# imazen/image-webp

Measured on AMD Instinct MI355X. Metric: 1920x1080 lossy encodes/s (Q75, method 4), higher is better.
Workload: dtype int32; 1 GPU; encode_frame_lossy 1920x1080 RGBA Q75 m4; device_batch=1024, distinct_frames=4, mbs_per_frame=8160, parallelism=frames sharded over 1 GPU(s), steps_pipelined=True, pipeline_lanes=2

## Files before the change

### image-webp_amd/csrc/zw_enc_kernels.hip

```cpp
#include "zw_dev.h"

#include <type_traits>

#include "zw_enc_rows.h"

#ifdef ZW_NW
#define ZW_NW1 ZW_NW
#define ZW_NW2 ZW_NW
#endif
#ifndef ZW_NW1
#define ZW_NW1 12
#endif
#ifndef ZW_NW2
#define ZW_NW2 12
#endif
#define NW_MAX (ZW_NW1 > ZW_NW2 ? ZW_NW1 : ZW_NW2)
#ifndef ZW_DYN_PRIO
#define ZW_DYN_PRIO 1
#endif
#ifndef ZW_DYN_PRIO1
#define ZW_DYN_PRIO1 2
#endif
#ifndef ZW_P1_LUMA_MAX
#define ZW_P1_LUMA_MAX 3
// ... 467 lines not shown
            for (int i = 0; i < 4; i++) accum[i] = dacc[i] = 0;
            int cc = 0;
            for (int a = min_a; a <= max_a; a++) {
                if (H[a] > 0) {
                    while (cc + 1 < 4) {
                        int dc = iabs(a - centers[cc]), dn = iabs(a - centers[cc + 1]);
                        if (dn < dc) cc++;
                        else break;
                    }
                    map[a] = (uint8_t)cc;
                    dacc[cc] += (uint32_t)a * H[a];
                    accum[cc] += H[a];
                }
            }
            int displaced = 0;
            wa = 0;
            tw = 0;
            for (int n = 0; n < 4; n++) {
                if (accum[n] > 0) {
                    uint8_t nc = (uint8_t)((dacc[n] + accum[n] / 2) / accum[n]);
                    displaced += iabs(centers[n] - nc);
                    centers[n] = nc;
                    wa += (int)nc * (int)accum[n];
                    tw += accum[n];
                }
            }
            if (displaced < 5) break;
        }
        int mid = tw > 0 ? (wa + (int)tw / 2) / (int)tw : 128;
        int minc = centers[0], maxc = centers[0];
        for (int i = 1; i < 4; i++) {
            minc = min(minc, (int)centers[i]);
            maxc = max(maxc, (int)centers[i]);
        }
        int rng = maxc == minc ? 1 : maxc - minc;
        for (int s = 0; s < 4; s++) {
            int ta = 255 * ((int)centers[s] - mid) / rng;
            ta = ta < -127 ? -127 : (ta > 127 ? 127 : ta);
            int sq = segment_quant(base, ta, 50);
            int delta = (int)(int8_t)((int8_t)sq - (int8_t)base);
            segment_init(P.seg[s], sq, delta);
        }
        uint32_t cnt[4] = {0, 0, 0, 0};
        for (int a = 0; a < 256; a++) cnt[map[a]] += H[a];
        uint32_t t01 = cnt[0] + cnt[1], t23 = cnt[2] + cnt[3];
#define GETP(a, b) ((a) + (b) == 0 ? 255 : (uint8_t)((255 * (a) + ((a) + (b)) / 2) / ((a) + (b))))
        P.seg_probs[0] = GETP(t01, t23);
        P.seg_probs[1] = GETP(cnt[0], cnt[1]);
        P.seg_probs[2] = GETP(cnt[2], cnt[3]);
#undef GETP
        P.seg_update_map = P.seg_probs[0] != 255 || P.seg_probs[1] != 255 || P.seg_probs[2] != 255;
        P.seg_enabled = 1;
    }
    params[f] = P;
    uint4* Hz = (uint4*)(histo + (size_t)f * 256);
    for (int i = 0; i < 64; i++) Hz[i] = make_uint4(0u, 0u, 0u, 0u);
}

struct EncArgs {
    const uint8_t *Y, *U, *V;
    const uint8_t* alpha;
    const ZwFrameParams* params;
    const ZwLevelCosts* lcost;
    int8_t* derr;
    ZwMbOut* out;
    uint8_t *ry, *ru, *rv;
    size_t ysz, csz;
    int mbw, mbh, pass;
    int* dbg;
    uint8_t* rows;
    uint32_t* sizes;
    int nframes;
};

struct MbLds {
    uint8_t sy[256], su[64], sv[64];
    uint8_t ws[17 * ZW_BPS];
    uint8_t left_y[20], left_u[12], left_v[12], left_c[12];
    int8_t left_derr[4];
    uint8_t modes[16];
    int16_t lev[25][16];
};

struct WaveLds {
    MbLds mb;
    uint8_t cu[9 * ZW_BPS], cv[9 * ZW_BPS];
    uint32_t uvc[64][8];
    int dc[64];
    int y2d[64];
    int y2cost[4];
    int V[2][40];
    int nzt[4], nzl[4];
    int misc[16];
    uint32_t pst[2][4];
    uint8_t win_y[32], win_u[8], win_v[8], win_c[12];
    int8_t win_d[4];
#ifdef ZW_PHASE_PROF
    unsigned long long ph[24];
#endif
};


struct Ctx {
    const EncArgs* a;
    const ZwFrameParams* P;
    int method;
    const ZwSegment* S;
    const ZwSegment* Sl;
    const LdsTables* T;
    WaveLds* W;
    MbLds* M;
    uint8_t *top_y, *top_u, *top_v, *top_c;
    int8_t* top_derr;
    const uint8_t *srcY, *srcU, *srcV;
    const uint8_t *sY, *sU, *sV;
    int ys, cs;
    int mbx, mby, lane, seg;
    int f;
    int oy, oc, ocx, od;
};

__device__ void build_luma_border(const Ctx& C, int part = 2)
{
    uint8_t* ws = C.M->ws;
    const int l = C.lane;
    const int mbw = C.a->mbw;
    const bool want = part == 2 || (part == 0 ? (l < 17 || l >= 32) : (l >= 17 && l < 32));
    if (!want) {
    } else if (l < 32) {
        int v;
        if (l == 0) v = C.mby == 0 ? 127 : (C.mbx == 0 ? 129 : C.M->left_y[0]);
        else if (C.mby == 0) v = 127;
        else if (l <= 16) v = C.top_y[C.oy + l - 1];
        else if (C.mbx == mbw - 1) v = C.top_y[C.oy + 15];
        else v = C.top_y[C.oy + l - 1];
        ws[l] = (uint8_t)v;
        if (l >= 17 && l < 21) {
            ws[4 * ZW_BPS + l] = (uint8_t)v;
            ws[8 * ZW_BPS + l] = (uint8_t)v;
            ws[12 * ZW_BPS + l] = (uint8_t)v;
        }
    } else if (l < 48) {
        int i = l - 32;
        ws[(i + 1) * ZW_BPS] = C.mbx == 0 ? 129 : C.M->left_y[1 + i];
    }
    wsync();
}

__device__ void build_chroma_border(const Ctx& C)
{
    const int l = C.lane;
    if (l < 34) {
        const int pl = l >= 17;
        const int i = pl ? l - 17 : l;
        uint8_t* w = pl ? C.W->cv : C.W->cu;
        const uint8_t* top = pl ? C.top_v : C.top_u;
        const uint8_t* left = pl ? C.M->left_v : C.M->left_u;
        if (i == 0) w[0] = C.mby == 0 ? 127 : (C.mbx == 0 ? 129 : left[0]);
        else if (i <= 8) w[i] = C.mby == 0 ? 127 : top[C.oc + i - 1];
        else w[(i - 8) * ZW_BPS] = C.mbx == 0 ? 129 : left[i - 8];
    }
    wsync();
}

template <int PASS>
__device__ void pick_i16(const Ctx& C, int& best_mode, unsigned long long& best_score)
{
    const int lane = C.lane, m = lane >> 4, b = lane & 15, bx = b & 3, by = b >> 2;
    const uint8_t* ws = C.M->ws;
    const ZwSegment& S = *C.S;
    const LdsTables* T = C.T;
    const int above = C.mby != 0, left = C.mbx != 0;
    int dcv;
    {
        const int top = lane < 16;
        const int v = (int)ws[csel(top, 1 + b, (b + 1) * ZW_BPS)] & -(int)(lane < 32 && (top ? above : left));
        const int sum = red16(v);
        const int s = __builtin_amdgcn_readlane(sum, 0) + __builtin_amdgcn_readlane(sum, 16);
        const int shf = 3 + above + left;
        dcv = (!above && !left) ? 128 : ((s + (1 << (shf - 1))) >> shf);
    }
    int src[16], pr[16], r[16], c[16];
    {
        const int P0 = ws[0];
        int L[4], Tp[4];
#pragma unroll
        for (int i = 0; i < 4; i++) {
            L[i] = ws[(by * 4 + i + 1) * ZW_BPS];
            Tp[i] = ws[1 + bx * 4 + i];
        }
#pragma unroll
        for (int i = 0; i < 4; i++) {
            const uint32_t srow = *(const uint32_t*)(C.sY + (by * 4 + i) * 16 + bx * 4);
#pragma unroll
            for (int j = 0; j < 4; j++) {
                const int p = sel4(m, dcv, Tp[j], L[i], clamp255(L[i] + Tp[j] - P0));
                const int sv = (int)((srow >> (8 * j)) & 255u);
                src[i * 4 + j] = sv;
                pr[i * 4 + j] = p;
                r[i * 4 + j] = sv - p;
            }
        }
    }
    fdct16_pk(r, c);
    int aq[16], dq[16];
    aq[0] = 0;
    int nzac = 0;
#pragma unroll
    for (int k = 1; k < 16; k++) {
        aq[k] = (int)((__umul24((uint32_t)iabs(c[k]), S.y1.iq[1]) + S.y1.bias[1]) >> 17);
        nzac |= aq[k];
        dq[k] = m24(c[k] < 0 ? -aq[k] : aq[k], (int)S.y1.q[1]);
    }
    nzac = nzac != 0;
    int cost = (int)rcost_bf<1, PASS == 2>(aq, 0, 0, T);
    int y2cost;
    {
        const int d = wht_g(c[0], b);
        const int t = b > 0;
        const int ay = (int)((__umul24((uint32_t)iabs(d), S.y2.iq[t]) + S.y2.bias[t]) >> 17);
        const int qy = d < 0 ? -ay : ay;
        y2cost = (int)rcost_g<0, PASS == 2>(qy, b, 0, 1, T);
        dq[0] = iwht_g(m24(qy, (int)S.y2.q[t]), b);
    }
    idct16(dq);
    int rec[16], sse = 0, flat = 1;
    const int s00 = C.sY[0];
#pragma unroll
    for (int k = 0; k < 16; k++) {
        rec[k] = clamp255(pr[k] + dq[k]);
        const int d = src[k] - rec[k];
        sse += m24(d, d);
        flat &= src[k] == s00;
    }
    int td = iabs(ttransform_diff_pk(rec, src)) >> 5;
    sse = red16(sse);
    td = red16(td);
    cost = red16(cost);
    nzac = red16(nzac);
    flat = red16(flat);
    const int srcflat = __builtin_amdgcn_readlane(flat, 0) == 16;
    cost += y2cost;
    int sd = S.tlambda > 0 ? ((int)S.tlambda * td + 128) >> 8 : 0;
    int dfin = sse;
    if (srcflat && nzac == 0) {
        dfin = sse * 2;
        sd = sd * 2;
    }
    const int mcost = sel4(m, d_FIXED_COSTS_I16[0], d_FIXED_COSTS_I16[1], d_FIXED_COSTS_I16[2], d_FIXED_COSTS_I16[3]) + cost;
    const int dist = dfin + sd;
    long long brd = 0x7fffffffffffffffLL, bfin = 0;
    int bm = 0;
#pragma unroll
    for (int mm = 0; mm < 4; mm++) {
        const long long mc = __builtin_amdgcn_readlane(mcost, mm * 16);
        const long long dd = 256LL * __builtin_amdgcn_readlane(dist, mm * 16);
        const long long r_m = mc * (long long)S.l_i16 + dd;
        const long long f_m = mc * (long long)S.l_mode + dd;
        const int avail = mm == 0 || (mm == 1 && above) || (mm == 2 && left) || (mm == 3 && above && left);
        if (avail && r_m < brd) {
            brd = r_m;
            bfin = f_m;
            bm = mm;
        }
    }
    best_mode = bm;
    best_score = bfin < 0 ? 0ull : (unsigned long long)bfin;
}

#ifdef ZW_PHASE_PROF
__device__ unsigned long long zw_phase_cycles_dev[2][24];
__device__ unsigned long long zw_wave_cycles_dev[2][16][24];
#define PH_START() long long ph_t_ = clock64()
#define PH_RESET() (ph_t_ = clock64())
#define PH_MARK(k) PH_MARK_L(k, lane, PASS)
#define PH_MARK_L(k, ln, ps)                                                        \
    do {                                                                            \
        const long long n_ = clock64();                                             \
        if ((ln) == 0) C.W->ph[k] += (unsigned long long)(n_ - ph_t_);               \
        ph_t_ = n_;                                                                 \
    } while (0)
extern "C" int zw_wave_cycles(unsigned long long* out, int reset)
{
    if (hipMemcpyFromSymbol(out, HIP_SYMBOL(zw_wave_cycles_dev), sizeof(zw_wave_cycles_dev)) != hipSuccess) return -1;
    if (reset) {
        static unsigned long long z[2][16][24];
        if (hipMemcpyToSymbol(HIP_SYMBOL(zw_wave_cycles_dev), z, sizeof z) != hipSuccess) return -1;
    }
    return 0;
}
extern "C" int zw_phase_cycles(unsigned long long* out, int reset)
{
    if (hipMemcpyFromSymbol(out, HIP_SYMBOL(zw_phase_cycles_dev), sizeof(zw_phase_cycles_dev)) != hipSuccess) return -1;
    if (reset) {
        static unsigned long long z[2][24];
        if (hipMemcpyToSymbol(HIP_SYMBOL(zw_phase_cycles_dev), z, sizeof z) != hipSuccess) return -1;
    }
    return 0;
}
#define PH_COUNT(k) \
    do {                \
        if (C.lane == 0) C.W->ph[k] += 1; \
    } while (0)
#elif defined(ZW_ASM_MARKS)
#define PH_COUNT(k) (void)0
#define PH_START() asm volatile("; ZWMARK start" ::: "memory")
#define PH_RESET() (void)0
#define PH_MARK(k) asm volatile("; ZWMARK " #k ::: "memory")
#define PH_MARK_L(k, ln, ps) asm volatile("; ZWMARK " #k ::: "memory")
#else
#define PH_COUNT(k) (void)0
#define PH_START() (void)0
#define PH_RESET() (void)0
#define PH_MARK(k) (void)0
#define PH_MARK_L(k, ln, ps) (void)0
#endif

template <int NB>
__device__ __forceinline__ void i4_values_n(const Ctx& C, const int* x0, const int* y0)
{
    WaveLds* W = C.W;
    const uint8_t* ws = C.M->ws;
    const int l = C.lane;
    const int t = (int)(l >= 13) + (int)(l >= 24) + (int)(l >= 36) + (int)(l >= 37);
    const int k = min(l - 13 * (int)(l >= 13) - 11 * (int)(l >= 24), 12);
    const int t3 = (int)(t == 3), t4 = (int)(t >= 4), t12 = (int)(t == 1 || t == 2);
    const int ka = k + t3 * (11 - k) + t4 * (1 - k);
    const int kb = k + t12 + t3 * (12 - k) - t4 * k;
    const int kc = min(k + 2 * (int)(t == 1), 12);
    const int wb = 2 * (int)(t == 1) + (int)(t == 2) + 3 * (t3 + t4);
    const int wc = (int)(t == 1);
    const int sh = (int)(t != 0) + (int)(t != 0 && t != 2);
    const int oa = csel(ka < 4, -ka * ZW_BPS, ka - 4 - 4 * ZW_BPS);
    const int ob = csel(kb < 4, -kb * ZW_BPS, kb - 4 - 4 * ZW_BPS);
    const int oc = csel(kc < 4, -kc * ZW_BPS, kc - 4 - 4 * ZW_BPS);
    const bool dcl = l < 4 || (l >= 5 && l < 9);
    int v[NB], ea[NB];
#pragma unroll
    for (int h = 0; h < NB; h++) {
        const int rowL = (y0[h] + 3) * ZW_BPS + x0[h] - 1;
        ea[h] = ws[rowL + oa];
        const int eb = ws[rowL + ob], ec = ws[rowL + oc];
        v[h] = (ea[h] + wb * eb + wc * ec + ((1 << sh) >> 1)) >> sh;
    }
#pragma unroll
    for (int h = 0; h < NB; h++) {
        const int dsum = red16(dcl ? ea[h] : 0);
        if (l < 38) W->V[h][l] = v[h];
        if (l == 0) W->V[h][38] = (dsum + 4) >> 3;
    }
// ... 906 lines not shown
    const unsigned long long win = __ballot(key2 == kmin);
    const uint32_t pk = (rate & 0xffffu) | ((uint32_t)mcost << 16) | ((uint32_t)(last >= 0) << 31);
    PH_MARK_L(12, l, 0);
#pragma unroll
    for (int mb = 0; mb < 2; mb++) {
        const ZwSegment& S = *(mb ? CB : CA).S;
        MbLds* M = (mb ? CB : CA).M;
#pragma unroll
        for (int h = 0; h < NB; h++) {
            const int gg = 2 * mb + h;
            const int bk = __builtin_ctz((uint32_t)(win >> (16 * gg)) & 0xffffu) >> 2;
            const int bmode = (int)((modes >> (16 * gg + 4 * bk)) & 15ull);
            const int wl = 16 * gg + 4 * bk;
            const uint32_t bsse = (uint32_t)__builtin_amdgcn_readlane(sse, wl);
            const uint32_t bpk = (uint32_t)__builtin_amdgcn_readlane((int)pk, wl);
            const uint32_t brate = bpk & 0xffffu;
            const int bnz = (int)(bpk >> 31);
            const int i = sby[h] * 4 + sbx[h];
            I4State& s = st[mb];
            s.tnz = (s.tnz & ~(1u << sbx[h])) | ((uint32_t)bnz << sbx[h]);
            s.lnz = (s.lnz & ~(1u << sby[h])) | ((uint32_t)bnz << sby[h]);
            s.nzm |= (uint32_t)bnz << i;
            s.total_mc += (bpk >> 16) & 0x7fffu;
            s.running += rdscore(bsse, brate, S.l_mode);
            s.mpack |= (unsigned long long)bmode << (4 * i);
            if (act[mb] && l == gg) M->modes[i] = (uint8_t)bmode;
        }
    }
    const int bks = __builtin_ctz((uint32_t)(win >> (16 * g)) & 0xffffu) >> 2;
    if (k == bks && ((l >> 4) & 1) < NB && (hm ? act[1] : act[0])) {
        MbLds* M = hm ? CB.M : CA.M;
        const int xo = csel(slot, x0[sl], x0[0]), yo = csel(slot, y0[sl], y0[0]);
        const uint32_t wd = __builtin_amdgcn_perm(r32, r01, 0x04060200u);
        uint8_t* p = M->ws + (yo + q) * ZW_BPS + xo;
#pragma unroll
        for (int j = 0; j < 4; j++) p[j] = (uint8_t)(wd >> (8 * j));
        if (keep) {
            int16_t* lvp = M->lev[by * 4 + bx];
#pragma unroll
            for (int r = 0; r < 4; r++) lvp[izz_of(4 * r + q)] = (int16_t)lv[r];
        }
    }
    wsync();
    PH_MARK_L(13, l, 0);
}

template <int PASS>
__device__ uint32_t pick_i4_pair(const Ctx& CA, const Ctx& CB, unsigned long long i16A, unsigned long long i16B,
                                 bool actA, bool actB, bool keep, uint32_t& nzA, uint32_t& nzB)
{
    const int K = CA.method <= 3 ? 3 : 4;
    I4State st[2];
    st[0].running = 211ull * CA.S->l_mode;
    st[1].running = 211ull * CB.S->l_mode;
#pragma unroll
    for (int mb = 0; mb < 2; mb++) {
        st[mb].total_mc = 0;
        st[mb].mpack = 0;
        st[mb].tnz = st[mb].lnz = st[mb].nzm = 0;
    }
    bool act[2] = {actA, actB};
    const unsigned long long lim[2] = {i16A, i16B};
    I4PLane LC;
    i4p_lane_init(CA, CB, LC);
    for (int s = 0; s < 10; s++) {
        const int sbyA = s < 4 ? 0 : (s - 2) >> 1;
        const int sbxA = s - 2 * sbyA;
        if (s >= 2 && s <= 7) {
            const int bx[2] = {sbxA, sbxA - 2}, by[2] = {sbyA, sbyA + 1};
            i4p_step<PASS, 2>(CA, CB, bx, by, K, LC, st, act, keep);
        } else {
            i4p_step<PASS, 1>(CA, CB, &sbxA, &sbyA, K, LC, st, act, keep);
        }
#pragma unroll
        for (int mb = 0; mb < 2; mb++)
            if (st[mb].running >= lim[mb] || st[mb].total_mc > 256u * 16u * 16u / 4u) act[mb] = false;
        if (!act[0] && !act[1]) return 0;
    }
    nzA = st[0].nzm;
    nzB = st[1].nzm;
    return (uint32_t)act[0] | ((uint32_t)act[1] << 1);
}

__device__ int final_luma(const Ctx& C, int mode, bool trel, int y_nz_out[16], int i4_nzm)
{
    WaveLds* W = C.W;
    const ZwSegment& S = *C.S;
    const int l = C.lane;
    int anynz = 0;
    PH_START();
    if (mode == 4 && i4_nzm >= 0) {
#pragma unroll
        for (int i = 0; i < 16; i++) y_nz_out[i] = (i4_nzm >> i) & 1;
        if (l < 16) C.M->lev[16][l] = 0;
        wsync();
        PH_MARK_L(15, l, 0);
        PH_COUNT(7);
        return i4_nzm != 0;
    }
    if (mode != 4) {
        build_luma_border(C);
        const uint8_t* ws = C.M->ws;
        const int above = C.mby != 0, left = C.mbx != 0;
        const int b = l & 15, bx = b & 3, by = b >> 2;
        int dcv;
        {
            const int top = l < 16;
            const int v = (int)ws[csel(top, 1 + b, (b + 1) * ZW_BPS)] & -(int)(l < 32 && (top ? above : left));
            const int sum = red16(v);
            const int su = __builtin_amdgcn_readlane(sum, 0) + __builtin_amdgcn_readlane(sum, 16);
            const int shf = 3 + above + left;
            dcv = (!above && !left) ? 128 : ((su + (1 << (shf - 1))) >> shf);
        }
        int c[16], pr[16];
        {
            const int P0 = ws[0];
            int L[4], Tp[4], r[16];
#pragma unroll
            for (int i = 0; i < 4; i++) {
                L[i] = ws[(by * 4 + i + 1) * ZW_BPS];
                Tp[i] = ws[1 + bx * 4 + i];
            }
#pragma unroll
            for (int i = 0; i < 4; i++) {
                const uint32_t srow = *(const uint32_t*)(C.sY + (by * 4 + i) * 16 + bx * 4);
#pragma unroll
                for (int j = 0; j < 4; j++) {
                    const int p = sel4(mode, dcv, Tp[j], L[i], clamp255(L[i] + Tp[j] - P0));
                    pr[i * 4 + j] = p;
                    r[i * 4 + j] = (int)((srow >> (8 * j)) & 255u) - p;
                }
            }
            fdct16_pk(r, c);
        }
        int y2dq;
        {
            const int d = wht_g(c[0], b);
            const int t = b > 0;
            const int y2q = quantz(d, S.y2.iq[t], S.y2.bias[t]);
            if (l < 16) C.M->lev[16][izz_of(b)] = (int16_t)y2q;
            if (gmask(y2q != 0)) anynz = 1;
            y2dq = iwht_g(m24(y2q, (int)S.y2.q[t]), b);
        }
        PH_MARK_L(16, l, 0);
        int dq[16], lv[16];
        int nzb = 0;
        {
            int snz = 0;
            if (l < 16) {
#pragma unroll
                for (int k = 1; k < 16; k++) snz |= quantz(c[k], S.y1.iq[1], S.y1.bias[1]) != 0;
            }
            anynz |= __any(snz) ? 1 : 0;
        }
        if (trel) {
            int tnz = 0;
            if (l < 48) {
#pragma unroll
                for (int k = 0; k < 16; k++) dq[k] = c[k];
                tnz = trellis<1, true>(dq, lv, S.y1, S.sharpen, S.lt_i16, C.T, 0, l >> 4);
            }
            PH_MARK_L(17, l, 0);
            const unsigned long long nzm = __ballot(l < 48 && tnz);
            int nt[4], nl[4];
#pragma unroll
            for (int q = 0; q < 4; q++) {
                nt[q] = __builtin_amdgcn_readfirstlane(C.top_c[C.ocx + 1 + q]);
                nl[q] = __builtin_amdgcn_readfirstlane(C.M->left_c[1 + q]);
            }
            unsigned code = 0, nzbits = 0;
#pragma unroll
            for (int bb = 0; bb < 16; bb++) {
                const int cx = min(nl[bb >> 2] + nt[bb & 3], 2);
                const int z = (int)((nzm >> (cx * 16 + bb)) & 1ull);
                nt[bb & 3] = z;
                nl[bb >> 2] = z;
                code |= (unsigned)cx << (2 * bb);
                nzbits |= (unsigned)z << bb;
            }
            const int srcl = (int)((code >> (2 * b)) & 3u) * 16 + b;
            lv[0] = 0;
#pragma unroll
            for (int i = 0; i < 8; i++) {
                const uint32_t w = (uint32_t)__shfl((int)pack_lo(lv[2 * i], lv[2 * i + 1]), srcl);
                lv[2 * i] = lo16(w);
                lv[2 * i + 1] = hi16(w);
            }
#pragma unroll
            for (int n = 1; n < 16; n++) dq[kZZ(n)] = m24(lv[n], (int)S.y1.q[1]);
            nzb = (nzbits >> b) & 1u;
            PH_MARK_L(18, l, 0);
        } else if (l < 16) {
#pragma unroll
            for (int n = 1; n < 16; n++) {
                const int j = kZZ(n);
                lv[n] = quantz(c[j], S.y1.iq[1], S.y1.bias[1]);
                nzb |= lv[n] != 0;
            }
            dq[0] = 0;
#pragma unroll
            for (int n = 1; n < 16; n++) dq[kZZ(n)] = m24(lv[n], (int)S.y1.q[1]);
        }
        wsync();
        if (l < 16) {
            lv[0] = 0;
#pragma unroll
            for (int n = 0; n < 16; n++) C.M->lev[b][n] = (int16_t)lv[n];
            dq[0] = y2dq;
            idct16(dq);
            uint8_t* wsp = C.M->ws;
#pragma unroll
            for (int k = 0; k < 16; k++) {
                const int y = by * 4 + (k >> 2), x = bx * 4 + (k & 3);
                wsp[(y + 1) * ZW_BPS + 1 + x] = (uint8_t)clamp255(pr[k] + dq[k]);
            }
        }
        const unsigned nzmask = (unsigned)__ballot(l < 16 && nzb);
        for (int k = 0; k < 16; k++) y_nz_out[k] = (int)((nzmask >> k) & 1u);
        wsync();
        PH_MARK_L(14, l, 0);
    } else {
        build_luma_border(C);
        int top_nz[4], left_nz[4];
        for (int k = 0; k < 4; k++) {
            top_nz[k] = C.top_c[C.ocx + 1 + k];
            left_nz[k] = C.M->left_c[1 + k];
        }
        for (int i = 0; i < 16; i++) {
            const int sby = i >> 2, sbx = i & 3, x0 = sbx * 4 + 1, y0 = sby * 4 + 1;
            const int bm = C.M->modes[i];
            i4_values(C, x0, y0);
            const int k = l & 15;
            const int pk = i4_pred_at(W->V[0], i4_src_index(C.T, bm, k), W->V[0][5 + (k & 3)] - W->V[0][4]);
            const int svk = C.sY[(sby * 4 + (k >> 2)) * 16 + sbx * 4 + (k & 3)];
            const int ck = fdct_g(svk - pk, k);
            const int ctx0 = min(left_nz[sby] + top_nz[sbx], 2);
            if (C.a->dbg && C.a->pass == 2 && l < 16) {
                int* d = C.a->dbg + (((size_t)C.f * C.a->mbw * C.a->mbh + (size_t)C.mby * C.a->mbw + C.mbx) * 16 + i) * 34;
                d[k] = ck;
                d[16 + k] = pk;
                if (k == 0) {
                    d[32] = ctx0;
                    d[33] = bm;
                }
            }
            const int qs = quantz(ck, S.y1.iq[k > 0], S.y1.bias[k > 0]);
            const int snz = gmask(qs != 0) != 0;
            int dqk, nzq;
            if (trel) {
                const int cn = gget(ck, zz_of(k));
                int lvn;
                nzq = trellis_g<0>(cn, k, S.y1, S.sharpen, S.lt_i4, C.T, 3, ctx0, lvn);
                if (l < 16) C.M->lev[i][k] = (int16_t)lvn;
                dqk = m24(gget(lvn, izz_of(k)), (int)S.y1.q[k > 0]);
            } else {
                if (l < 16) C.M->lev[i][izz_of(k)] = (int16_t)qs;
                nzq = snz;
                dqk = m24(qs, (int)S.y1.q[k > 0]);
            }
            const int rk = idct_g(dqk, k);
            if (l < 16) C.M->ws[(y0 + (k >> 2)) * ZW_BPS + x0 + (k & 3)] = (uint8_t)clamp255(pk + rk);
            wsync();
            if (l == 0) {
                W->misc[1] = nzq;
                W->misc[2] = snz;
            }
            wsync();
            const int nz = W->misc[1];
            anynz |= W->misc[2];
            top_nz[sbx] = nz;
            left_nz[sby] = nz;
            y_nz_out[i] = nz;
            wsync();
        }
        if (l < 16) C.M->lev[16][l] = 0;
        wsync();
        PH_MARK_L(15, l, 0);
        PH_COUNT(7);
    }
    return anynz;
}

__device__ int final_chroma(const Ctx& C, int mode, int8_t* top_derr, int uv_nz[8])
{
    WaveLds* W = C.W;
    const ZwSegment& S = *C.S;
    const int l = C.lane;
    const int h = l >> 5, b = l & 7, pl = b >> 2, bx = b & 1, by = (b >> 1) & 1;
    const bool act = (l & 31) < 8;
    int cf[2][4];
    uint32_t p01[2], p32[2];
    {
        const uint32_t* e = W->uvc[h * 32 + mode * 8 + b];
#pragma unroll
        for (int c = 0; c < 2; c++) {
            cf[c][0] = lo16(e[2 * c]);
            cf[c][1] = hi16(e[2 * c]);
            cf[c][2] = lo16(e[2 * c + 1]);
            cf[c][3] = hi16(e[2 * c + 1]);
        }
        p01[0] = e[4];
        p32[0] = e[5];
        p01[1] = e[6];
        p32[1] = e[7];
    }
    {
        const int q = (int)S.uv.q[0];
        const uint32_t iq = S.uv.iq[0], bias = S.uv.bias[0];
        const uint32_t zt = S.uv.zthresh[0];
        int dcs[8];
#pragma unroll
        for (int k = 0; k < 8; k++) dcs[k] = __builtin_amdgcn_readlane(cf[0][0], k);
        auto diffuse = [&](int& dc, int te, int le) -> int {
            dc += (7 * te + 8 * le) >> 3;
            const int sign = dc < 0;
            const uint32_t a = (uint32_t)(sign ? -dc : dc);
            const int level = a > zt ? (int)((a * iq + bias) >> 17) : 0;
            const int err = (int)a - level * q;
            const int se = sign ? -err : err;
            const int v = se >> 1;
            return (int)(int8_t)(v < -127 ? -127 : (v > 127 ? 127 : v));
        };
#pragma unroll
        for (int ch = 0; ch < 2; ch++) {
            int8_t* top = top_derr + ch * 2;
            int8_t* lft = C.M->left_derr + ch * 2;
            const int t0 = __builtin_amdgcn_readfirstlane((int)top[0]), t1 = __builtin_amdgcn_readfirstlane((int)top[1]);
            const int l0 = __builtin_amdgcn_readfirstlane((int)lft[0]), l1 = __builtin_amdgcn_readfirstlane((int)lft[1]);
            int* d = dcs + ch * 4;
            const int e0 = diffuse(d[0], t0, l0);
            const int e1 = diffuse(d[1], t1, e0);
            const int e2 = diffuse(d[2], e0, l1);
            const int e3 = diffuse(d[3], e1, e2);
            const int nl1 = (int)(int8_t)((3 * e3) >> 2);
            wsync();
            if (l == 0) {
                lft[0] = (int8_t)e1;
                lft[1] = (int8_t)nl1;
                top[0] = (int8_t)e2;
                top[1] = (int8_t)(e3 - nl1);
            }
        }
#pragma unroll
        for (int k = 0; k < 8; k++)
            asm volatile("v_writelane_b32 %0, %1, %2" : "+v"(cf[0][0]) : "s"(__builtin_amdgcn_readfirstlane(dcs[k])), "i"(k));
    }
    int dq[2][4];
    int nz = 0;
#pragma unroll
    for (int c = 0; c < 2; c++)
#pragma unroll
        for (int r = 0; r < 4; r++) {
            const bool dcs = c == 0 && r == 0;
            const uint32_t iq = dcs ? (h ? S.uv.iq[1] : S.uv.iq[0]) : S.uv.iq[1];
            const uint32_t bias = dcs ? (h ? S.uv.bias[1] : S.uv.bias[0]) : S.uv.bias[1];
// ... 645 lines not shown
                    C.mbx = mbx;
                    C.mby = mby;
                    if (lane < 16) ((uint32_t*)C.M->su)[lane] = cur.y;
                    wsync();
                    const int seg = __builtin_amdgcn_readfirstlane((int)seg_lut[cur.alpha]);
                    C.seg = seg;
                    C.S = C.Sl + seg;
                    uvq_border(C, U);
                    const int cm = uvq_pick(C, U, xch, xflag, ++seq);
                    PH_MARK(8);
                    uvq_final(C, U, cm, top_derr + mbx * 4);
                    PH_MARK(9);
                    uvq_store_borders(C, U);
                    ZwMbOut* o = a.out + (size_t)f * nmb + (size_t)mby * mbw + mbx;
                    if (pl == 0 && lane == 0) o->chroma_mode = (uint8_t)cm;
                    write_levels(C, 17 + 4 * pl, 4, false);
                    wsync();
                }
            }
            for (int i = lane; i < mbw * 2; i += 64) {
                const int j = (i >> 1) * 4 + pl * 2 + (i & 1);
                a.derr[(size_t)f * mbw * 4 + j] = top_derr[j];
            }
            ph_flush();
            return;
        }
        MbFetch nx = fetch_mb(&a, fc, lane, 0, 0);
        for (int mby = 0; has_chain && mby < mbh; mby++) {
            if (lane < 12) {
                C.M->left_u[lane] = 129;
                C.M->left_v[lane] = 129;
            }
            wsync();
            for (int mbx = 0; mbx < mbw; mbx++) {
                PH_START();
                const int lane = opaque_lane(threadIdx.x & 63);
                C.lane = lane;
                const MbFetch cur = nx;
                if (mbx + 1 < mbw) nx = fetch_mb(&a, fc, lane, mbx + 1, mby);
                else if (mby + 1 < mbh) nx = fetch_mb(&a, fc, lane, 0, mby + 1);
                setup_ctx(C, &a, lutc, W, mbx, mby, cur);
                C.oc = mbx * 8;
                C.ocx = mbx * 12;
                build_chroma_border(C);
                const int cm = pick_uv<PASS>(C);
                PH_MARK(8);
                int uvnz[8];
                final_chroma(C, cm, tdc + mbx * 4, uvnz);
                PH_MARK(9);
                store_chroma_borders(C);
                ZwMbOut* o = a.out + (size_t)fc * nmb + (size_t)mby * mbw + mbx;
                if (lane == 0) o->chroma_mode = (uint8_t)cm;
                write_levels(C, 17, 8, false);
                wsync();
            }
        }
        for (int i = lane; has_chain && i < mbw * 4; i += 64) a.derr[(size_t)fc * mbw * 4 + i] = tdc[i];
        if (!PAIR) {
            ph_flush();
            return;
        }
        C.f = f;
        C.P = P;
        C.T = T;
        C.Sl = Sl;
        C.top_u = top_u;
        C.top_v = top_v;
        C.top_derr = top_derr;
        C.method = __builtin_amdgcn_readfirstlane(P->method);
    }

    if (PASS == 1) __builtin_amdgcn_s_setprio(ZW_LUMA_PRIO);
    using RS = RowSchedule<PASS, ROWS, NW, NCH>;
    constexpr bool skip_mode = RS::skip_mode;
    constexpr int nrw = RS::nrw;
    const int rw = ROWS ? 0 : RS::first_row(wv, mbh);
    if (ROWS) {
        C.top_y = W->win_y;
        C.top_u = W->win_u;
        C.top_v = W->win_v;
        C.top_c = W->win_c;
        C.top_derr = W->win_d;
    }
    auto mb_store = [&](Ctx& C, int lm, int cm, bool i4reuse, uint32_t i4nz, bool trel) __attribute__((always_inline)) {
        const int lane = C.lane;
        PH_START();
        int ynz[16];
        const int lnz = final_luma(C, lm, trel, ynz, i4reuse ? (int)i4nz : -1);
        PH_MARK(4);
        int uvnz[8] = {0, 0, 0, 0, 0, 0, 0, 0};
        int cnz = 0;
        if (PASS == 2) cnz = final_chroma(C, cm, C.top_derr + C.od, uvnz);
        PH_MARK(5);
        ZwMbOut* o = a.out + (size_t)C.f * nmb + (size_t)C.mby * mbw + C.mbx;
        if (PASS == 2) {
            const int skip = !(lnz | cnz);
            if (lane == 0) {
                uint8_t* tc = C.top_c + C.ocx;
                uint8_t* lc = C.M->left_c;
                if (skip) {
                    for (int k = 1; k < 9; k++) tc[k] = lc[k] = 0;
                    if (lm != 4) tc[0] = lc[0] = 0;
                } else {
                    if (lm != 4) {
                        int y2nz = 0;
                        for (int n = 0; n < 16; n++) y2nz |= C.M->lev[16][n] != 0;
                        tc[0] = lc[0] = (uint8_t)y2nz;
                    }
                    for (int x = 0; x < 4; x++) tc[1 + x] = (uint8_t)ynz[12 + x];
                    for (int y = 0; y < 4; y++) lc[1 + y] = (uint8_t)ynz[y * 4 + 3];
                    tc[5] = (uint8_t)uvnz[2];
                    tc[6] = (uint8_t)uvnz[3];
                    lc[5] = (uint8_t)uvnz[1];
                    lc[6] = (uint8_t)uvnz[3];
                    tc[7] = (uint8_t)uvnz[6];
                    tc[8] = (uint8_t)uvnz[7];
                    lc[7] = (uint8_t)uvnz[5];
                    lc[8] = (uint8_t)uvnz[7];
                }
                o->skip = (uint8_t)skip;
                o->chroma_mode = (uint8_t)cm;
            }
            store_chroma_borders(C);
            write_levels(C, 0, 25, skip);
            if (a.sizes) {
                int e = 0;
                if (lane < 25 && !skip) {
                    const uint32_t* lw = (const uint32_t*)C.M->lev[lane];
#pragma unroll
                    for (int q = 0; q < 8; q++) {
                        const uint32_t v = lw[q];
                        e = (v >> 16) ? 2 * q + 2 : ((v & 0xffffu) ? 2 * q + 1 : e);
                    }
                }
                const int r16 = red16(e);
                const int es = __builtin_amdgcn_readlane(r16, 0) + __builtin_amdgcn_readlane(r16, 16);
                if (lane == 0)
                    a.sizes[(size_t)C.f * nmb + (size_t)C.mby * mbw + C.mbx] = (uint32_t)(1 + (lm == 4 ? 8 : 0) + 25 + 2 * es);
            }
        } else {
            write_levels(C, 0, 17, false);
            if (lane == 0) o->skip = 0;
        }
        if (lane == 0) {
            o->luma_mode = (uint8_t)lm;
            o->segment = (uint8_t)C.seg;
        }
        if (lane < 16) o->bpred[lane] = lm == 4 ? C.M->modes[lane] : 0;
        store_luma_borders(C);
    };
    if constexpr (PAIR) {
        MbLds* const Mp[2] = {&W->mb, Mall2 + wv};
        const int meth0 = C.method;
        const int K = C.method <= 3 ? 3 : (C.method == 4 ? 4 : 10);
        const int meth1 = nf == 2 ? __builtin_amdgcn_readfirstlane(a.params[f + 1].method) : C.method;
        const bool trel1 = PASS == 2 && nf == 2 && __builtin_amdgcn_readfirstlane(a.params[f + 1].do_trellis);
        const bool keep1 = !trel1 && (PASS == 1 || a.dbg == nullptr);
        using RP =
            typename std::conditional<PASS == 1, PairRowSchedule1<NW, NCW>, RowSchedule<PASS, ROWS, NW, NCW, true>>::type;
        const bool same_k = nf == 1 || (meth1 == C.method && trel1 == trel);
        for (int mby = RP::first_row(wv, mbh); mby < mbh; mby = RP::next_row(wv, mby, mbh)) {
#pragma unroll
            for (int fr = 0; fr < 2; fr++) row_start(Mp[fr], lane);
            wsync();
            const int prevw = mby > 0 ? RP::wave_of_row(mby - 1, mbh) : 0;
            auto wait_above = [&](int need) {
                if (mby > 0) wait_row(progress, prevw, (mby - 1) * 65536 + need);
            };
            for (int mbx = 0; mbx < mbw; mbx++) {
                PH_START();
                const int lane = opaque_lane(threadIdx.x & 63);
                C.lane = lane;
                auto enter = [&](int fr) {
                    C.lane = opaque_lane(threadIdx.x & 63);
                    C.f = f + fr;
                    C.P = a.params + C.f;
                    C.T = (const LdsTables*)((const uint8_t*)T + L.sT * fr);
                    C.Sl = (const ZwSegment*)((const uint8_t*)Sl + L.sS * fr);
                    C.top_y = top_y + L.sy * fr;
                    C.top_u = top_u + L.su * fr;
                    C.top_v = top_v + L.sv * fr;
                    C.top_c = top_c + L.sc * fr;
                    C.top_derr = top_derr + L.sd * fr;
                    C.M = fr ? Mp[1] : Mp[0];
                    C.method = fr ? meth1 : meth0;
                    C.mbx = mbx;
                    C.mby = mby;
                    C.oy = mbx * 16;
                    C.oc = mbx * 8;
                    C.ocx = mbx * 12;
                    C.od = mbx * 4;
                    C.sY = C.M->sy;
                    C.sU = C.M->su;
                    C.sV = C.M->sv;
                };
                auto pst = [&](int fr, int k) { return (uint32_t)__builtin_amdgcn_readfirstlane((int)W->pst[fr][k]); };
                wait_above(min(mbx + 1, mbw));
                luma_issue_prio<PASS>(progress, prevw, mbx, mby, mbw);
                PH_MARK(0);
ZW_PAIR_LOOP
                for (int fr = 0; fr < 2; fr++) {
                    if (fr >= nf) {
                        if (lane == 0) W->pst[fr][0] = 0;
                        continue;
                    }
                    enter(fr);
                    const MbFetch fm = fetch_mb(&a, C.f, lane, mbx, mby);
                    setup_ctx(C, &a, seg_lut + L.sL * fr, W, mbx, mby, fm);
                    build_luma_border(C, 0);
                    int l_;
                    unsigned long long s_;
                    pick_i16<PASS>(C, l_, s_);
                    const bool n_ = C.method > 1 && (C.method >= 5 || s_ > 211ull * C.S->l_mode || l_ != 0);
                    if (lane == 0) {
                        W->pst[fr][0] = (uint32_t)l_ | ((uint32_t)n_ << 4) | ((uint32_t)C.seg << 8);
                        W->pst[fr][1] = (uint32_t)s_;
                        W->pst[fr][2] = (uint32_t)(s_ >> 32);
                        W->pst[fr][3] = 0;
                    }
                    wsync();
                }
                wsync();
                PH_MARK(1);
                const uint32_t s0 = pst(0, 0), s1 = pst(1, 0);
                const bool n0 = (s0 >> 4) & 1u, n1 = (s1 >> 4) & 1u;
                if (n0 || n1) wait_above(min(mbx + 2, mbw));
ZW_PAIR_LOOP
                for (int fr = 0; fr < 2; fr++) {
                    if (!((pst(fr, 0) >> 4) & 1u)) continue;
                    enter(fr);
                    build_luma_border(C, 1);
                }
                PH_MARK(21);
                if (K <= 4 && same_k && (n0 || n1)) {
                    Ctx CA = C, CB = C;
                    CA.lane = CB.lane = opaque_lane(threadIdx.x & 63);
                    CA.T = T;
                    CB.T = (const LdsTables*)((const uint8_t*)T + L.sT);
                    CA.M = Mp[0];
                    CB.M = Mp[1];
                    CA.S = Sl + (s0 >> 8);
                    CB.S = (const ZwSegment*)((const uint8_t*)Sl + L.sS) + (s1 >> 8);
                    CA.sY = Mp[0]->sy;
                    CB.sY = Mp[1]->sy;
                    const unsigned long long i0 = pst(0, 1) | ((unsigned long long)pst(0, 2) << 32);
                    const unsigned long long i1 = pst(1, 1) | ((unsigned long long)pst(1, 2) << 32);
                    uint32_t z0 = 0, z1 = 0;
                    const uint32_t r = pick_i4_pair<PASS>(CA, CB, i0, i1, n0, n1, keep_i4, z0, z1);
                    if (lane == 0) {
                        W->pst[0][3] = (r & 1u) ? (z0 | 0x10000u) : 0u;
                        W->pst[1][3] = (r & 2u) ? (z1 | 0x10000u) : 0u;
                    }
                } else if (n0 || n1) {
ZW_PAIR_LOOP
                    for (int fr = 0; fr < 2; fr++) {
                        const uint32_t sm = pst(fr, 0);
                        if (!((sm >> 4) & 1u)) continue;
                        enter(fr);
                        C.seg = (int)(sm >> 8);
                        C.S = C.Sl + C.seg;
                        uint32_t z = 0;
                        const bool w4 = pick_i4<PASS>(C, pst(fr, 1) | ((unsigned long long)pst(fr, 2) << 32),
                                                      fr ? keep1 : keep_i4, z);
                        if (lane == 0) W->pst[fr][3] = w4 ? (z | 0x10000u) : 0u;
                    }
                }
                wsync();
                PH_MARK(2);
ZW_PAIR_LOOP
                for (int fr = 0; fr < 2; fr++) {
                    if (fr >= nf) continue;
                    enter(fr);
                    const uint32_t sm = pst(fr, 0), r4 = pst(fr, 3);
                    C.seg = (int)(sm >> 8);
                    C.S = C.Sl + C.seg;
                    int cm = 0;
                    if (PASS == 2) {
                        build_chroma_border(C);
                        cm = pick_uv<PASS>(C);
                    }
                    PH_MARK(3);
                    const bool w4 = (r4 >> 16) & 1u;
                    mb_store(C, w4 ? 4 : (int)(sm & 15u), cm, w4 && (fr ? keep1 : keep_i4), r4 & 0xffffu,
                             fr ? trel1 : trel);
                    PH_RESET();
                }
                publish(progress, wv, mby * 65536 + mbx + 1);
                PH_MARK(6);
            }
        }
        ph_flush();
        return;
    }
    uint8_t* const gty = ROWS ? rb + RL.ty : nullptr;
    uint8_t* const gtu = ROWS ? rb + RL.tu : nullptr;
    uint8_t* const gtv = ROWS ? rb + RL.tv : nullptr;
    uint8_t* const gtc = ROWS ? rb + RL.tc : nullptr;
    uint8_t* const gtd = ROWS ? rb + RL.td : nullptr;
    for (int it = 0, yk = rw;; it++) {
        const int mby = ROWS ? row_ticket(&rsync[0]) : (skip_mode ? yk : rw + it * nrw);
        if (skip_mode) yk = RS::next_row(wv, yk, mbh);
        if (mby >= mbh) break;
        row_start(C.M, lane);
        wsync();
        const int prevw = (!ROWS && mby > 0) ? RS::wave_of_row(mby - 1) : 0;
        int seen = -1;
        int* const prog_above = ROWS ? rsync + 4 + (mby > 0 ? mby - 1 : 0) : nullptr;
        auto wait_above = [&](int need) {
            if (mby == 0) return;
            if (ROWS) row_wait(prog_above, need, rerr, seen);
            else wait_row(progress, prevw, (mby - 1) * 65536 + need);
        };
        MbFetch nx;
        if (ZW_FETCH_AHEAD) nx = fetch_mb(&a, f, lane, 0, mby);
        for (int mbx = 0; mbx < mbw; mbx++) {
            PH_START();
            const int lane = opaque_lane(threadIdx.x & 63);
            C.lane = lane;
            MbFetch cur;
            if (ZW_FETCH_AHEAD) {
                cur = nx;
                if (mbx + 1 < mbw) nx = fetch_mb(&a, f, lane, mbx + 1, mby);
            } else {
                cur = fetch_mb(&a, f, lane, mbx, mby);
            }
            wait_above(min(mbx + 1, mbw));
            if (ROWS) {
                if (mby > 0) {
                    uint32_t v = 0;
                    if (lane < 4) v = ld_sc1(gty + mbx * 16 + 4 * lane);
                    else if (PASS == 2 && lane < 6) v = ld_sc1(gtu + mbx * 8 + 4 * (lane - 4));
                    else if (PASS == 2 && lane < 8) v = ld_sc1(gtv + mbx * 8 + 4 * (lane - 6));
                    else if (PASS == 2 && lane < 11) v = ld_sc1(gtc + mbx * 12 + 4 * (lane - 8));
                    else if (PASS == 2 && lane < 12) v = ld_sc1(gtd + mbx * 4);
                    if (lane < 4) ((uint32_t*)W->win_y)[lane] = v;
                    else if (PASS == 2 && lane < 6) ((uint32_t*)W->win_u)[lane - 4] = v;
                    else if (PASS == 2 && lane < 8) ((uint32_t*)W->win_v)[lane - 6] = v;
                    else if (PASS == 2 && lane < 11) ((uint32_t*)W->win_c)[lane - 8] = v;
                    else if (PASS == 2 && lane < 12) ((uint32_t*)W->win_d)[0] = v;
                } else if (PASS == 2) {
                    if (lane < 3) ((uint32_t*)W->win_c)[lane] = 0;
                    else if (lane == 3)
                        ((uint32_t*)W->win_d)[0] = *(const uint32_t*)(a.derr + (size_t)f * mbw * 4 + mbx * 4);
                }
                wsync();
            } else {
                C.oy = mbx * 16;
                C.oc = mbx * 8;
                C.ocx = mbx * 12;
                C.od = mbx * 4;
            }
            if (!ROWS) luma_issue_prio<PASS>(progress, prevw, mbx, mby, mbw);
            PH_MARK(0);
            setup_ctx(C, &a, seg_lut, W, mbx, mby, cur);
            build_luma_border(C, 0);
            int lm;
            unsigned long long i16s;
            pick_i16<PASS>(C, lm, i16s);
            wsync();
            PH_MARK(1);
            int cm = 0;
            uint32_t i4nz = 0;
            bool i4reuse = false;
            if (PASS == 2) {
                build_chroma_border(C);
                cm = pick_uv<PASS>(C);
            }
            PH_MARK(3);
            if (C.method > 1) {
                const unsigned long long thr = 211ull * C.S->l_mode;
                if (C.method >= 5 || i16s > thr || lm != 0) {
                    wait_above(min(mbx + 2, mbw));
                    if (ROWS && mby > 0 && mbx + 1 < mbw) {
                        uint32_t v = 0;
                        if (lane < 4) v = ld_sc1(gty + (mbx + 1) * 16 + 4 * lane);
                        if (lane < 4) ((uint32_t*)W->win_y)[4 + lane] = v;
                        wsync();
                    }
                    build_luma_border(C, 1);
                    PH_MARK(21);
                    if (pick_i4<PASS>(C, i16s, keep_i4, i4nz)) {
                        lm = 4;
                        i4reuse = keep_i4;
                    }
                }
            }
            PH_MARK(2);
            mb_store(C, lm, cm, i4reuse, i4nz, trel);
            PH_RESET();
            if (ROWS) {
                if (mby + 1 < mbh) {
                    if (lane < 4) st_sc1(gty + mbx * 16 + 4 * lane, ((const uint32_t*)W->win_y)[lane]);
                    else if (PASS == 2 && lane < 6) st_sc1(gtu + mbx * 8 + 4 * (lane - 4), ((const uint32_t*)W->win_u)[lane - 4]);
                    else if (PASS == 2 && lane < 8) st_sc1(gtv + mbx * 8 + 4 * (lane - 6), ((const uint32_t*)W->win_v)[lane - 6]);
                    else if (PASS == 2 && lane < 11) st_sc1(gtc + mbx * 12 + 4 * (lane - 8), ((const uint32_t*)W->win_c)[lane - 8]);
                    else if (PASS == 2 && lane < 12) st_sc1(gtd + mbx * 4, ((const uint32_t*)W->win_d)[0]);
                    row_publish(rsync + 4 + mby, mbx + 1);
                }
            } else {
                publish(progress, wv, mby * 65536 + mbx + 1);
            }
            PH_MARK(6);
        }
    }
    ph_flush();
}

extern "C" __global__ __launch_bounds__(PassShape<1>::WG) void k_encode_pass1(EncArgs a) { encode_body<1, false>(a); }
extern "C" __global__ __launch_bounds__(PassShape<1>::WG) void k_encode_pass1_fp(EncArgs a) { encode_body<1, false, 2>(a); }
extern "C" __global__ __launch_bounds__(PassShape<2>::WG) void k_encode_pass2(EncArgs a) { encode_body<2, false>(a); }
extern "C" __global__ __launch_bounds__(PassShape<2>::WG) void k_encode_pass2_fp(EncArgs a) { encode_body<2, false, 2>(a); }
extern "C" __global__ __launch_bounds__(64 * RowsShape<1>::NW) void k_encode_rows_pass1(EncArgs a) { encode_body<1, true>(a); }
extern "C" __global__ __launch_bounds__(64) void k_encode_rows_pass2(EncArgs a) { encode_body<2, true>(a); }

struct QuantBlocksArgs {
    ZwMatrix m;
    uint16_t sharpen[16];
    uint32_t lambda;
    int32_t ctype, first, trel, n;
};

extern "C" __global__ __launch_bounds__(256) void k_quant_blocks(const int* __restrict__ coeffs,
                                                                const uint8_t* __restrict__ ctx0s,
                                                                const ZwLevelCosts* __restrict__ lcost,
                                                                const uint8_t* __restrict__ probs, QuantBlocksArgs a,
                                                                int* __restrict__ levels, int* __restrict__ dq)
{
    __shared__ LdsTables T;
    for (int i = threadIdx.x; i < (int)(sizeof(T.lc) / 2); i += 256) (&T.lc[0][0][0][0])[i] = (&lcost->lc[0][0][0][0])[i];
    for (int i = threadIdx.x; i < 96; i += 256) {
        (&T.eob[0][0][0])[i] = (&lcost->eob[0][0][0])[i];
        (&T.init[0][0][0])[i] = (&lcost->init[0][0][0])[i];
    }
    for (int i = threadIdx.x; i < 4 * 8 * 3 * 11; i += 256) (&T.probs[0][0][0][0])[i] = probs[i];
    load_static_tables(&T, threadIdx.x, 256, probs);
    __syncthreads();
    const int b = blockIdx.x * 256 + threadIdx.x;
    if (b >= a.n) return;
    int c[16], lv[16];
#pragma unroll
    for (int k = 0; k < 16; k++) c[k] = coeffs[(size_t)b * 16 + k];
    const int ctx0 = ctx0s[b];
    if (a.trel) {
        if (a.first) trellis<1>(c, lv, a.m, a.sharpen, a.lambda, &T, a.ctype, ctx0);
        else trellis<0>(c, lv, a.m, a.sharpen, a.lambda, &T, a.ctype, ctx0);
        if (a.first) lv[0] = 0;
    } else {
#pragma unroll
        for (int n = 0; n < 16; n++) {
            const int j = kZZ(n);
            lv[n] = n < a.first ? 0 : quantz(c[j], a.m.iq[j > 0], a.m.bias[j > 0]);
        }
#pragma unroll
        for (int n = 0; n < 16; n++) {
            const int j = kZZ(n);
            c[j] = n < a.first ? 0 : m24(lv[n], (int)a.m.q[j > 0]);
        }
    }
#pragma unroll
    for (int k = 0; k < 16; k++) {
        levels[(size_t)b * 16 + k] = lv[k];
        dq[(size_t)b * 16 + k] = c[k];
    }
}

extern "C" __global__ __launch_bounds__(256) void k_quant_blocks_g(const int* __restrict__ coeffs,
                                                                  const uint8_t* __restrict__ ctx0s,
                                                                  const ZwLevelCosts* __restrict__ lcost,
                                                                  const uint8_t* __restrict__ probs, QuantBlocksArgs a,
                                                                  int* __restrict__ levels, int* __restrict__ dq)
{
// ... 166 lines not shown
```

Baseline: 4485 encodes/s.

## Stash winning I16 coefficients and prediction in LDS to skip recompute in final_luma

pick_i16 now writes the winning mode's quantized (or, for trellis, raw) coefficients, the Y2 level and the packed predicted or reconstructed pixels into LDS. final_luma reuses them instead of rebuilding the border, predicting and running the forward DCT again, and for non-trellis it copies levels and reconstruction straight through. final_luma is also moved out of mb_store into its own loop in the paired-MB path, with the nz mask passed as a bitmask. This adds LDS writes on every pick_i16 call and reuses the uvc area as stash space in the paired lane, which relies on uvc not being live at that point.

```diff
diff --git a/image-webp_amd/csrc/zw_enc_kernels.hip b/image-webp_amd/csrc/zw_enc_kernels.hip
--- a/image-webp_amd/csrc/zw_enc_kernels.hip
+++ b/image-webp_amd/csrc/zw_enc_kernels.hip
@@ -573,15 +573,14 @@
     int16_t lev[25][16];
 };
 
+constexpr int I16_STASH = 16 * 8 + 1;
+
 struct WaveLds {
     MbLds mb;
     uint8_t cu[9 * ZW_BPS], cv[9 * ZW_BPS];
     uint32_t uvc[64][8];
-    int dc[64];
-    int y2d[64];
-    int y2cost[4];
+    uint32_t i16c[I16_STASH + 11];
     int V[2][40];
-    int nzt[4], nzl[4];
     int misc[16];
     uint32_t pst[2][4];
     uint8_t win_y[32], win_u[8], win_v[8], win_c[12];
@@ -611,6 +610,14 @@
     int oy, oc, ocx, od;
 };
 
+DI uint32_t* i16_stash(const Ctx& C) { return C.M == &C.W->mb ? C.W->i16c : &C.W->uvc[0][0]; }
+DI uint32_t* i16_stash_px(const Ctx& C) { return (uint32_t*)&C.M->lev[17][0]; }
+DI uint32_t pack_px(const int* p)
+{
+    return (uint32_t)p[0] | ((uint32_t)p[1] << 8) | ((uint32_t)p[2] << 16) | ((uint32_t)p[3] << 24);
+}
+static_assert(sizeof(((WaveLds*)0)->uvc) >= I16_STASH * 4 && offsetof(MbLds, lev) % 4 == 0, "the I16 hand-over");
+
 __device__ void build_luma_border(const Ctx& C, int part = 2)
 {
     uint8_t* ws = C.M->ws;
@@ -655,7 +662,7 @@
 }
 
 template <int PASS>
-__device__ void pick_i16(const Ctx& C, int& best_mode, unsigned long long& best_score)
+__device__ void pick_i16(const Ctx& C, bool trel, int& best_mode, unsigned long long& best_score)
 {
     const int lane = C.lane, m = lane >> 4, b = lane & 15, bx = b & 3, by = b >> 2;
     const uint8_t* ws = C.M->ws;
@@ -694,18 +701,25 @@
         }
     }
     fdct16_pk(r, c);
-    int aq[16], dq[16];
+    int aq[16], dq[16], sl[16];
     aq[0] = 0;
     int nzac = 0;
 #pragma unroll
     for (int k = 1; k < 16; k++) {
         aq[k] = (int)((__umul24((uint32_t)iabs(c[k]), S.y1.iq[1]) + S.y1.bias[1]) >> 17);
         nzac |= aq[k];
-        dq[k] = m24(c[k] < 0 ? -aq[k] : aq[k], (int)S.y1.q[1]);
+        sl[k] = c[k] < 0 ? -aq[k] : aq[k];
+        dq[k] = m24(sl[k], (int)S.y1.q[1]);
     }
     nzac = nzac != 0;
+    uint32_t hw[8], hp[4];
+#pragma unroll
+    for (int i = 1; i < 8; i++) {
+        if (PASS == 2 && trel) hw[i] = pack_lo(c[2 * i], c[2 * i + 1]);
+        else hw[i] = pack_lo(sl[kZZ(2 * i)], sl[kZZ(2 * i + 1)]);
+    }
     int cost = (int)rcost_bf<1, PASS == 2>(aq, 0, 0, T);
-    int y2cost;
+    int y2cost, snz;
     {
         const int d = wht_g(c[0], b);
         const int t = b > 0;
@@ -713,6 +727,8 @@
         const int qy = d < 0 ? -ay : ay;
         y2cost = (int)rcost_g<0, PASS == 2>(qy, b, 0, 1, T);
         dq[0] = iwht_g(m24(qy, (int)S.y2.q[t]), b);
+        hw[0] = pack_lo(qy, (PASS == 2 && trel) ? c[1] : sl[1]);
+        snz = nzac | (ay != 0);
     }
     idct16(dq);
     int rec[16], sse = 0, flat = 1;
@@ -723,6 +739,11 @@
         const int d = src[k] - rec[k];
         sse += m24(d, d);
         flat &= src[k] == s00;
+    }
+#pragma unroll
+    for (int i = 0; i < 4; i++) {
+        if (PASS == 2 && trel) hp[i] = pack_px(pr + 4 * i);
+        else hp[i] = pack_px(rec + 4 * i);
     }
     int td = iabs(ttransform_diff_pk(rec, src)) >> 5;
     sse = red16(sse);
@@ -757,6 +778,19 @@
     }
     best_mode = bm;
     best_score = bfin < 0 ? 0ull : (unsigned long long)bfin;
+    {
+        uint32_t* st = i16_stash(C);
+        uint32_t* sp = i16_stash_px(C);
+        const bool win = m == bm;
+        const bool anynz = __ballot(win && snz) != 0ull;
+        if (win) {
+#pragma unroll
+            for (int i = 0; i < 8; i++) st[i * 16 + b] = hw[i];
+#pragma unroll
+            for (int i = 0; i < 4; i++) sp[i * 16 + b] = hp[i];
+            if (b == 0) st[128] = anynz;
+        }
+    }
 }
 
 #ifdef ZW_PHASE_PROF
@@ -1829,7 +1863,7 @@
     return (uint32_t)act[0] | ((uint32_t)act[1] << 1);
 }
 
-__device__ int final_luma(const Ctx& C, int mode, bool trel, int y_nz_out[16], int i4_nzm)
+__device__ int final_luma(const Ctx& C, int mode, bool trel, uint32_t& y_nzm, int i4_nzm)
 {
     WaveLds* W = C.W;
     const ZwSegment& S = *C.S;
@@ -1837,70 +1871,66 @@
     int anynz = 0;
     PH_START();
     if (mode == 4 && i4_nzm >= 0) {
-#pragma unroll
-        for (int i = 0; i < 16; i++) y_nz_out[i] = (i4_nzm >> i) & 1;
+        y_nzm = (uint32_t)i4_nzm;
         if (l < 16) C.M->lev[16][l] = 0;
         wsync();
         PH_MARK_L(15, l, 0);
         PH_COUNT(7);
         return i4_nzm != 0;
     }
-    if (mode != 4) {
-        build_luma_border(C);
-        const uint8_t* ws = C.M->ws;
-        const int above = C.mby != 0, left = C.mbx != 0;
+    if (mode != 4 && !trel) {
+        const uint32_t* st = i16_stash(C);
+        const int b = l & 15;
+        anynz = __builtin_amdgcn_readfirstlane((int)st[128]);
+        int nzb = 0;
+        if (l < 16) {
+            uint32_t w[8];
+#pragma unroll
+            for (int i = 0; i < 8; i++) w[i] = st[i * 16 + b];
+            C.M->lev[16][izz_of(b)] = (int16_t)lo16(w[0]);
+            w[0] &= 0xffff0000u;
+            uint32_t* lw = (uint32_t*)C.M->lev[b];
+            uint32_t any = 0;
+#pragma unroll
+            for (int i = 0; i < 8; i++) {
+                lw[i] = w[i];
+                any |= w[i];
+            }
+            nzb = any != 0u;
+        }
+        {
+            const uint32_t v = i16_stash_px(C)[l];
+            uint8_t* p = C.M->ws + ((b >> 2) * 4 + (l >> 4) + 1) * ZW_BPS + 1 + (b & 3) * 4;
+#pragma unroll
+            for (int j = 0; j < 4; j++) p[j] = (uint8_t)(v >> (8 * j));
+        }
+        y_nzm = (uint32_t)__ballot(l < 16 && nzb) & 0xffffu;
+        wsync();
+        PH_MARK_L(16, l, 0);
+    } else if (mode != 4) {
+        const uint32_t* st = i16_stash(C);
         const int b = l & 15, bx = b & 3, by = b >> 2;
-        int dcv;
-        {
-            const int top = l < 16;
-            const int v = (int)ws[csel(top, 1 + b, (b + 1) * ZW_BPS)] & -(int)(l < 32 && (top ? above : left));
-            const int sum = red16(v);
-            const int su = __builtin_amdgcn_readlane(sum, 0) + __builtin_amdgcn_readlane(sum, 16);
-            const int shf = 3 + above + left;
-            dcv = (!above && !left) ? 128 : ((su + (1 << (shf - 1))) >> shf);
-        }
-        int c[16], pr[16];
-        {
-            const int P0 = ws[0];
-            int L[4], Tp[4], r[16];
-#pragma unroll
-            for (int i = 0; i < 4; i++) {
-                L[i] = ws[(by * 4 + i + 1) * ZW_BPS];
-                Tp[i] = ws[1 + bx * 4 + i];
-            }
-#pragma unroll
-            for (int i = 0; i < 4; i++) {
-                const uint32_t srow = *(const uint32_t*)(C.sY + (by * 4 + i) * 16 + bx * 4);
-#pragma unroll
-                for (int j = 0; j < 4; j++) {
-                    const int p = sel4(mode, dcv, Tp[j], L[i], clamp255(L[i] + Tp[j] - P0));
-                    pr[i * 4 + j] = p;
-                    r[i * 4 + j] = (int)((srow >> (8 * j)) & 255u) - p;
-                }
-            }
-            fdct16_pk(r, c);
-        }
+        anynz = __builtin_amdgcn_readfirstlane((int)st[128]);
+        int c[16];
         int y2dq;
         {
-            const int d = wht_g(c[0], b);
-            const int t = b > 0;
-            const int y2q = quantz(d, S.y2.iq[t], S.y2.bias[t]);
+            uint32_t w[8];
+#pragma unroll
+            for (int i = 0; i < 8; i++) w[i] = st[i * 16 + b];
+#pragma unroll
+            for (int i = 0; i < 8; i++) {
+                c[2 * i] = lo16(w[i]);
+                c[2 * i + 1] = hi16(w[i]);
+            }
+            const int y2q = c[0];
+            c[0] = 0;
             if (l < 16) C.M->lev[16][izz_of(b)] = (int16_t)y2q;
-            if (gmask(y2q != 0)) anynz = 1;
-            y2dq = iwht_g(m24(y2q, (int)S.y2.q[t]), b);
+            y2dq = iwht_g(m24(y2q, (int)S.y2.q[b > 0]), b);
         }
         PH_MARK_L(16, l, 0);
         int dq[16], lv[16];
         int nzb = 0;
         {
-            int snz = 0;
-            if (l < 16) {
-#pragma unroll
-                for (int k = 1; k < 16; k++) snz |= quantz(c[k], S.y1.iq[1], S.y1.bias[1]) != 0;
-            }
-            anynz |= __any(snz) ? 1 : 0;
-        }
-        if (trel) {
             int tnz = 0;
             if (l < 48) {
 #pragma unroll
@@ -1937,38 +1967,29 @@
             for (int n = 1; n < 16; n++) dq[kZZ(n)] = m24(lv[n], (int)S.y1.q[1]);
             nzb = (nzbits >> b) & 1u;
             PH_MARK_L(18, l, 0);
-        } else if (l < 16) {
-#pragma unroll
-            for (int n = 1; n < 16; n++) {
-                const int j = kZZ(n);
-                lv[n] = quantz(c[j], S.y1.iq[1], S.y1.bias[1]);
-                nzb |= lv[n] != 0;
-            }
-            dq[0] = 0;
-#pragma unroll
-            for (int n = 1; n < 16; n++) dq[kZZ(n)] = m24(lv[n], (int)S.y1.q[1]);
-        }
-        wsync();
+        }
         if (l < 16) {
             lv[0] = 0;
 #pragma unroll
             for (int n = 0; n < 16; n++) C.M->lev[b][n] = (int16_t)lv[n];
             dq[0] = y2dq;
             idct16(dq);
+            const uint32_t* sp = i16_stash_px(C);
             uint8_t* wsp = C.M->ws;
 #pragma unroll
             for (int k = 0; k < 16; k++) {
                 const int y = by * 4 + (k >> 2), x = bx * 4 + (k & 3);
-                wsp[(y + 1) * ZW_BPS + 1 + x] = (uint8_t)clamp255(pr[k] + dq[k]);
+                const int pk = (int)((sp[(k >> 2) * 16 + b] >> (8 * (k & 3))) & 255u);
+                wsp[(y + 1) * ZW_BPS + 1 + x] = (uint8_t)clamp255(pk + dq[k]);
             }
         }
-        const unsigned nzmask = (unsigned)__ballot(l < 16 && nzb);
-        for (int k = 0; k < 16; k++) y_nz_out[k] = (int)((nzmask >> k) & 1u);
+        y_nzm = (uint32_t)__ballot(l < 16 && nzb) & 0xffffu;
         wsync();
         PH_MARK_L(14, l, 0);
     } else {
         build_luma_border(C);
         int top_nz[4], left_nz[4];
+        y_nzm = 0;
         for (int k = 0; k < 4; k++) {
             top_nz[k] = C.top_c[C.ocx + 1 + k];
             left_nz[k] = C.M->left_c[1 + k];
@@ -2017,7 +2038,7 @@
             anynz |= W->misc[2];
             top_nz[sbx] = nz;
             left_nz[sby] = nz;
-            y_nz_out[i] = nz;
+            y_nzm |= (uint32_t)(nz != 0) << i;
             wsync();
         }
         if (l < 16) C.M->lev[16][l] = 0;
@@ -2829,12 +2850,9 @@
         C.top_c = W->win_c;
         C.top_derr = W->win_d;
     }
-    auto mb_store = [&](Ctx& C, int lm, int cm, bool i4reuse, uint32_t i4nz, bool trel) __attribute__((always_inline)) {
+    auto mb_store = [&](Ctx& C, int lm, int cm, int lnz, uint32_t ynzm) __attribute__((always_inline)) {
         const int lane = C.lane;
         PH_START();
-        int ynz[16];
-        const int lnz = final_luma(C, lm, trel, ynz, i4reuse ? (int)i4nz : -1);
-        PH_MARK(4);
         int uvnz[8] = {0, 0, 0, 0, 0, 0, 0, 0};
         int cnz = 0;
         if (PASS == 2) cnz = final_chroma(C, cm, C.top_derr + C.od, uvnz);
@@ -2854,8 +2872,8 @@
                         for (int n = 0; n < 16; n++) y2nz |= C.M->lev[16][n] != 0;
                         tc[0] = lc[0] = (uint8_t)y2nz;
                     }
-                    for (int x = 0; x < 4; x++) tc[1 + x] = (uint8_t)ynz[12 + x];
-                    for (int y = 0; y < 4; y++) lc[1 + y] = (uint8_t)ynz[y * 4 + 3];
+                    for (int x = 0; x < 4; x++) tc[1 + x] = (uint8_t)((ynzm >> (12 + x)) & 1u);
+                    for (int y = 0; y < 4; y++) lc[1 + y] = (uint8_t)((ynzm >> (y * 4 + 3)) & 1u);
                     tc[5] = (uint8_t)uvnz[2];
                     tc[6] = (uint8_t)uvnz[3];
                     lc[5] = (uint8_t)uvnz[1];
@@ -2957,7 +2975,7 @@
                     build_luma_border(C, 0);
                     int l_;
                     unsigned long long s_;
-                    pick_i16<PASS>(C, l_, s_);
+                    pick_i16<PASS>(C, fr ? trel1 : trel, l_, s_);
                     const bool n_ = C.method > 1 && (C.method >= 5 || s_ > 211ull * C.S->l_mode || l_ != 0);
                     if (lane == 0) {
                         W->pst[fr][0] = (uint32_t)l_ | ((uint32_t)n_ << 4) | ((uint32_t)C.seg << 8);
@@ -3021,15 +3039,28 @@
                     const uint32_t sm = pst(fr, 0), r4 = pst(fr, 3);
                     C.seg = (int)(sm >> 8);
                     C.S = C.Sl + C.seg;
+                    const bool w4 = (r4 >> 16) & 1u;
+                    uint32_t ynzm;
+                    const int lnz = final_luma(C, w4 ? 4 : (int)(sm & 15u), fr ? trel1 : trel, ynzm,
+                                               w4 && (fr ? keep1 : keep_i4) ? (int)(r4 & 0xffffu) : -1);
+                    if (lane == 0) W->pst[fr][3] = ynzm | (r4 & 0x10000u) | ((uint32_t)(lnz != 0) << 17);
+                    PH_MARK(4);
+                }
+                wsync();
+ZW_PAIR_LOOP
+                for (int fr = 0; fr < 2; fr++) {
+                    if (fr >= nf) continue;
+                    enter(fr);
+                    const uint32_t sm = pst(fr, 0), r4 = pst(fr, 3);
+                    C.seg = (int)(sm >> 8);
+                    C.S = C.Sl + C.seg;
                     int cm = 0;
                     if (PASS == 2) {
                         build_chroma_border(C);
                         cm = pick_uv<PASS>(C);
                     }
                     PH_MARK(3);
-                    const bool w4 = (r4 >> 16) & 1u;
-                    mb_store(C, w4 ? 4 : (int)(sm & 15u), cm, w4 && (fr ? keep1 : keep_i4), r4 & 0xffffu,
-                             fr ? trel1 : trel);
+                    mb_store(C, ((r4 >> 16) & 1u) ? 4 : (int)(sm & 15u), cm, (int)((r4 >> 17) & 1u), r4 & 0xffffu);
                     PH_RESET();
                 }
                 publish(progress, wv, mby * 65536 + mbx + 1);
@@ -3103,7 +3134,7 @@
             build_luma_border(C, 0);
             int lm;
             unsigned long long i16s;
-            pick_i16<PASS>(C, lm, i16s);
+            pick_i16<PASS>(C, trel, lm, i16s);
             wsync();
             PH_MARK(1);
             int cm = 0;
@@ -3133,7 +3164,10 @@
                 }
             }
             PH_MARK(2);
-            mb_store(C, lm, cm, i4reuse, i4nz, trel);
+            uint32_t ynzm;
+            const int lnz = final_luma(C, lm, trel, ynzm, i4reuse ? (int)i4nz : -1);
+            PH_MARK(4);
+            mb_store(C, lm, cm, lnz, ynzm);
             PH_RESET();
             if (ROWS) {
                 if (mby + 1 < mbh) {
```

Measured after the change: 4344 encodes/s. 0.969x the previous value.
